# ekimb/rust-mdbg

Hardware: AMD Instinct MI355X
Metric: Gbases/s ingested to k-min-mer graph (higher is better)
Workload: dtype u64

## Files before the change

rust_mdbg_amd/csrc/owner.hip:

```cpp
#include "mdbg_dev.h"
__global__ void owner_thresholds_kernel(double bound, u32 k, u32 world, u64* __restrict__ thr) {
    const u32 r = threadIdx.x + 1;
    if (threadIdx.x == 0) thr[0] = 0;
    thr += OWNER_THR_AT;
    if (r >= world) return;
    const double x = -expm1(log1p(-(double)r / (double)world) / (double)k);
    double v = x * bound;
    thr[r - 1] = v >= 18446744073709549568.0 ? ~0ull : (u64)v;
}
void launch_owner_thresholds(double bound, u32 k, u32 world, u64* thr, hipStream_t s) {
    if (world > 1) hipLaunchKernelGGL(owner_thresholds_kernel, dim3(1), dim3(64), 0, s, bound, k, world, thr);
}

__global__ __launch_bounds__(256) void count_owned_windows_kernel(const u64* __restrict__ mh, const u32* __restrict__ mread, const u64* __restrict__ roff, u64 i0, u64 i1,
                                                                  u32 k, u32 world, const u64* thr, u32 rank, u64* __restrict__ out) {
    constexpr int WPT = 4;
    const u64 b0 = i0 + (u64)blockIdx.x * (256 * WPT);
    u32 slot[WPT]; bool ok[WPT];
#pragma unroll
    for (int u = 0; u < WPT; ++u) { const u64 i = b0 + u * 256 + threadIdx.x; ok[u] = i < i1; slot[u] = ok[u] ? mread[i] : 0; }
    u32 mine = 0;
#pragma unroll
    for (int u = 0; u < WPT; ++u) {
        const u64 i = b0 + u * 256 + threadIdx.x;
// ... 79 lines not shown
    if (threadIdx.x < world) hist[threadIdx.x] = 0;
    const u64 b0 = i0 + (u64)blockIdx.x * OWNL_SPAN;
    const OwnerSpec os{world, thr};
    const bool staged = k <= OWNL_LDS_MAX_K && thr != nullptr && world > 1;
    OwnerCodes oc{}; const u16* cur = nullptr; u32 p = 1;
    if (staged) {
        oc = owner_codes_of(os);
        u16* const ca = (u16*)sh_min;
        cur = span_min_codes([&](u32 t) { return mh[b0 + t]; }, [&](u32 t) { return b0 + t < i1; }, OWNL_SPAN + k - 1, k, oc, ca, ca + (OWNL_SPAN + k), p);
    } else __syncthreads();
#pragma unroll
    for (int u = 0; u < OWNL_SPAN / 256; ++u) {
        const u32 li = u * 256 + threadIdx.x;
        const u64 i = b0 + li;
        u32 o = 0xFFu;
        if (window_starts_at(mread, roff, i, i1, k)) {
            if (staged) { const u16 x = cur[li], y = cur[li + k - p]; o = owner_of_code(x < y ? x : y, oc); }
            else o = window_owner(mh + i, k, os);
            atomicAdd(&hist[o], 1u);
        }
        if (i < i1) owner_of[i - i0] = (u8)o;
    }
    __syncthreads();
    if (threadIdx.x < world) blk_cnt[(size_t)blockIdx.x * world + threadIdx.x] = hist[threadIdx.x];
}
void launch_owner_list_count(const u64* mh, const u32* mread, const u64* roff, u64 i0, u64 i1, u32 k, u32 world, const u64* thr, u32* blk_cnt, u8* owner_of, hipStream_t s) {
    if (i1 > i0) hipLaunchKernelGGL(owner_list_count_kernel, dim3((unsigned)((i1 - i0 + OWNL_SPAN - 1) / OWNL_SPAN)), dim3(256), owner_span_codes_lds(k), s, mh, mread, roff, i0, i1, k, world, thr, blk_cnt, owner_of);
}
__global__ __launch_bounds__(256) void owner_list_write_kernel(const u64* __restrict__ mh, const u32* __restrict__ mread, const u64* __restrict__ roff, u64 i0, u64 i1,
                                                               u32 k, u32 world, const u64* thr, u32 slot0, const u64* __restrict__ blk_off, OwnerBases bases, u32* __restrict__ list,
                                                               const u8* __restrict__ owner_of, u32 direct_owner, u32* __restrict__ direct_dst) {
    constexpr int NG = OWNL_SPAN / 64;
    __shared__ u32 grp[NG][OWNL_MAX_WORLD];
    for (int t = threadIdx.x; t < NG * (int)OWNL_MAX_WORLD; t += 256) ((u32*)grp)[t] = 0;
    __syncthreads();
    const u64 b0 = i0 + (u64)blockIdx.x * OWNL_SPAN;
    const int lane = threadIdx.x & 63, wv = threadIdx.x >> 6;
    constexpr u32 NONE = 0xFFFFFFFFu;
    u32 own[OWNL_SPAN / 256], rank[OWNL_SPAN / 256], slot_of[OWNL_SPAN / 256];
#pragma unroll
    for (int u = 0; u < OWNL_SPAN / 256; ++u) {
        const u64 i = b0 + u * 256 + threadIdx.x;
        u32 o = NONE, slot = 0;
        if (i < i1) { const u32 ob = owner_of[i - i0]; if (ob != 0xFFu) { o = ob; slot = mread[i]; } }
        u32 r = 0;
        for (u64 todo = __ballot(o != NONE); todo;) {
            const u32 oo = (u32)__shfl((int)o, __ffsll((unsigned long long)todo) - 1, 64);
            const u64 m = __ballot(o == oo);
            if (o == oo) { r = (u32)__popcll(m & ((1ull << lane) - 1)); if (r == 0) grp[u * 4 + wv][oo] = (u32)__popcll(m); }
            todo &= ~m;
        }
        own[u] = o; rank[u] = r; slot_of[u] = slot;
    }
    __syncthreads();
    if (threadIdx.x < world) { u32 run = 0; for (int g = 0; g < NG; ++g) { const u32 c = grp[g][threadIdx.x]; grp[g][threadIdx.x] = run; run += c; } }
    __syncthreads();
#pragma unroll
    for (int u = 0; u < OWNL_SPAN / 256; ++u) {
        const u32 o = own[u];
        if (o == NONE || (o == direct_owner && !direct_dst)) continue;
        const u64 i = b0 + u * 256 + threadIdx.x;
        const u64 at = blk_off[(size_t)blockIdx.x * world + o] + grp[u * 4 + wv][o] + rank[u];
        uint2* const e = o == direct_owner ? (uint2*)direct_dst + at : (uint2*)list + (bases.b[o] + at);
        *e = make_uint2((u32)(i - i0), slot_of[u] - slot0);
    }
}
void launch_owner_list_write(const u64* mh, const u32* mread, const u64* roff, u64 i0, u64 i1, u32 k, u32 world, const u64* thr, u32 slot0, const u64* blk_off, const OwnerBases& bases, u32* list, const u8* owner_of, hipStream_t s,
                             u32 direct_owner = 0xFFFFFFFFu, u32* direct_dst = nullptr) {
    if (i1 > i0) hipLaunchKernelGGL(owner_list_write_kernel, dim3((unsigned)((i1 - i0 + OWNL_SPAN - 1) / OWNL_SPAN)), dim3(256), 0, s, mh, mread, roff, i0, i1, k, world, thr, slot0, blk_off, bases, list, owner_of, direct_owner, direct_dst);
}

struct SegBuckets { u64 start[OWNL_MAX_WORLD + 1]; u64 base[OWNL_MAX_WORLD]; u64 lim[OWNL_MAX_WORLD]; u32 n; u32 skip; };
__device__ inline u32 seg_bucket_of(const SegBuckets& B, u64 j) {
    u32 lo = 0, hi = B.n - 1;
    while (lo < hi) { const u32 mid = (lo + hi + 1) >> 1; if (B.start[mid] <= j) lo = mid; else hi = mid - 1; }
    return lo;
}
__device__ inline u32 seg_add_of(const uint2* __restrict__ list, u64 j, u32 k, const SegBuckets& B, u32& b) {
    b = seg_bucket_of(B, j);
    if (b == B.skip) return 0;
    if (j && B.start[b] != j) { const u32 d = list[j].x - list[j - 1].x; if (d < k) return d; }
    return k;
}
constexpr u32 SEG_BLOCK = 4096;
__global__ __launch_bounds__(256) void seg_sums_kernel(const uint2* __restrict__ list, u64 n, u32 k, SegBuckets B, u64* __restrict__ block_sum) {
    __shared__ u32 ws[4];
    u32 v = 0;
#pragma unroll
    for (int q = 0; q < SEG_BLOCK / 256; ++q) { const u64 j = (u64)blockIdx.x * SEG_BLOCK + q * 256 + threadIdx.x; u32 b; if (j < n) v += seg_add_of(list, j, k, B, b); }
    for (int d = 32; d; d >>= 1) v += __shfl_down(v, d, 64);
    if ((threadIdx.x & 63) == 0) ws[threadIdx.x >> 6] = v;
    __syncthreads();
    if (threadIdx.x == 0) block_sum[blockIdx.x] = (u64)ws[0] + ws[1] + ws[2] + ws[3];
}
__global__ __launch_bounds__(256) void seg_pick_kernel(const uint2* __restrict__ list, u64 n, u32 k, SegBuckets B, const u64* __restrict__ block_base, const u64* __restrict__ total,
                                                       u64* __restrict__ out) {
    __shared__ u32 ws[4];
    const u32 bq = blockIdx.x;
    const u64 j1 = bq < B.n ? B.start[bq] : n;
    if (j1 >= n) { if (threadIdx.x == 0) out[bq] = total[0]; return; }
    const u64 j0 = j1 - j1 % SEG_BLOCK;
    u32 v = 0;
#pragma unroll
    for (int q = 0; q < SEG_BLOCK / 256; ++q) { const u64 j = j0 + q * 256 + threadIdx.x; u32 b; if (j < j1) v += seg_add_of(list, j, k, B, b); }
    for (int d = 32; d; d >>= 1) v += __shfl_down(v, d, 64);
    if ((threadIdx.x & 63) == 0) ws[threadIdx.x >> 6] = v;
    __syncthreads();
    if (threadIdx.x == 0) out[bq] = block_base[j0 / SEG_BLOCK] + ws[0] + ws[1] + ws[2] + ws[3];
}
void launch_seg_prefix(const u32* list, u64 n, u32 k, const SegBuckets& B, u64* scan_tmp, u64* carry, u64* picks, hipStream_t s) {
    if (!n) return;
    const u32 nb = (u32)((n + SEG_BLOCK - 1) / SEG_BLOCK);
    hipLaunchKernelGGL(seg_sums_kernel, dim3(nb), dim3(256), 0, s, (const uint2*)list, n, k, B, scan_tmp);
    hipLaunchKernelGGL(tile_scan_top_kernel, dim3(1), dim3(256), 0, s, nb, scan_tmp, carry);
    hipLaunchKernelGGL(seg_pick_kernel, dim3(B.n + 1), dim3(256), 0, s, (const uint2*)list, n, k, B, scan_tmp, carry, picks);
}
__global__ __launch_bounds__(256) void seg_copy_kernel(const uint2* __restrict__ list, u64 n, u32 k, SegBuckets B, const u64* __restrict__ block_base,
                                                       u64* __restrict__ store, u64* __restrict__ payload, u64 payload_n, u32 to_store) {
    __shared__ u32 lpre[256];
    __shared__ u64 laddr[256];
    __shared__ u32 tmp[8];
    u64 P0 = block_base[blockIdx.x];
#pragma unroll 1
    for (int q = 0; q < SEG_BLOCK / 256; ++q) {
        const u64 j = (u64)blockIdx.x * SEG_BLOCK + q * 256 + threadIdx.x;
        u32 a = 0, b = 0, x = 0;
        if (j < n) { a = seg_add_of(list, j, k, B, b); x = list[j].x; }
        u32 T;
        const u32 excl = block_excl_scan_256(a, tmp, T);
        u64 at = ~0ull;
        if (j < n && !((u64)x + k > B.lim[b] || P0 + excl + a > payload_n)) at = B.base[b] + x + (k - a);
        lpre[threadIdx.x] = j < n ? excl : 0xFFFFFFFFu;
        laddr[threadIdx.x] = at;
        __syncthreads();
        for (u32 e = threadIdx.x; e < T; e += 256) {
            u32 lo = 0, hi = 255;
#pragma unroll
            for (int st = 0; st < 8; ++st) { const u32 mid = (lo + hi + 1) >> 1; if (lpre[mid] <= e) lo = mid; else hi = mid - 1; }
            const u64 src = laddr[lo];
            if (src == ~0ull) continue;
            u64* const h = store + src + (e - lpre[lo]);
            u64* const pp = payload + P0 + e;
            if (to_store) *h = *pp; else *pp = *h;
        }
        P0 += T;
    }
}
void launch_seg_copy(const u32* list, u64 n, u32 k, const SegBuckets& B, const u64* scan_tmp, u64* store, u64* payload, u64 payload_n, bool to_store, hipStream_t s) {
    if (n) hipLaunchKernelGGL(seg_copy_kernel, dim3((unsigned)((n + SEG_BLOCK - 1) / SEG_BLOCK)), dim3(256), 0, s, (const uint2*)list, n, k, B, scan_tmp, store, payload, payload_n, to_store ? 1u : 0u);
}

__device__ inline bool listed_check(u64 j) { return (((u32)j * 0x9E3779B1u) >> 28) == 0; }
struct ListedBatch { u64 start, m0, m1, first_ordinal; const u32* list; u32 slot0, n_reads; };
__global__ __launch_bounds__(256) void insert_listed_entries_kernel(TableArgs T, const u64* __restrict__ mh, u32* __restrict__ mread, const u64* __restrict__ roff,
                                                                    u64 m0, u64 m1, const u32* __restrict__ list, u64 n, u32 slot0, u32 n_reads, u64 first_ordinal,
                                                                    u32* __restrict__ cap_err, const ListedBatch* __restrict__ multi, u32 n_multi) {
    if (cap_err[1]) return;
    const u64 j = (u64)blockIdx.x * blockDim.x + threadIdx.x;
    const u32 k = T.ks.k;
    bool ok = j < n;
    u64 i = 0, rs = 0; u32 slot = 0;
    u64 jl = j;
    if (multi) {
        const u64 jw0 = (u64)blockIdx.x * blockDim.x + (threadIdx.x & ~63u);
        u64 jw = ((u64)__builtin_amdgcn_readfirstlane((u32)(jw0 >> 32)) << 32) | (u64)__builtin_amdgcn_readfirstlane((u32)jw0);
        if (jw >= n) jw = n - 1;
        u32 lo = 0, hi = n_multi - 1;
        while (lo < hi) { const u32 mid = (lo + hi + 1) >> 1; if (multi[mid].start <= jw) lo = mid; else hi = mid - 1; }
        if (ok && multi[lo + 1].start <= j) {
            hi = n_multi - 1;
            while (lo < hi) { const u32 mid = (lo + hi + 1) >> 1; if (multi[mid].start <= j) lo = mid; else hi = mid - 1; }
        }
        const ListedBatch b = multi[lo];
        m0 = b.m0; m1 = b.m1; list = b.list; slot0 = b.slot0; n_reads = b.n_reads; first_ordinal = b.first_ordinal; jl = j - b.start;
    }
    if (ok) {
        const uint2 e = ((const uint2*)list)[jl];
        i = m0 + e.x; slot = slot0 + e.y; ok = e.y < n_reads && i + k <= m1;
    }
    const u64* const w = mh + i;
    bool rev = false; u64 h = 0;
    if (ok) {
        const u64 w_first = w[0], w_last = w[k - 1];
        rs = roff[slot]; const u64 re = roff[slot + 1];
        ok = i >= rs && re - rs > k && i + k <= re;
        if (ok) {
            rev = w_first != w_last ? w_first > w_last : window_reversed(w, k);
            u64 smallest;
            h = key_hash_window_hbm(w, k, rev, smallest);
            ok = owner_of_min(smallest, k, OwnerSpec{T.own_world, T.own_thr}) == T.own_rank;
        }
    }
    wave_count_add(ok, T.own_inserted);
    const u64 win = i - rs;
    if (ok && win > WIN_MASK) { *cap_err = 1; ok = false; }
    const u64 ord = ((first_ordinal + (slot - slot0)) << WIN_BITS) | win;
    bool claimed, found;
    const u64 s = upsert_wave_h(T, ok, (u32)i, i, w, k, rev, h, claimed, found);
    if (claimed) { mread[i] = slot; if (T.claim) T.claim[i] = 1; }
    if (found) {
        atomicAdd(&T.tab[s].count, 1u);
        push_ordinal(T, s, ord);
    }
}
static void launch_listed_entries(const TableArgs& T, const u64* mh, u32* mread, const u64* roff, u64 m0, u64 m1, const u32* list, u64 n, u32 slot0, u32 n_reads, u64 first_ordinal,
                                  u32* cap_err, const ListedBatch* multi, u32 n_multi, hipStream_t s) {
    hipLaunchKernelGGL(insert_listed_entries_kernel, dim3((unsigned)((n + 255) / 256)), dim3(256), 0, s, T, mh, mread, roff, m0, m1, list, n, slot0, n_reads, first_ordinal, cap_err, multi, n_multi);
}
__global__ __launch_bounds__(256) void list_segments_kernel(const u32* __restrict__ list, u64 n, u32 n_spans, u32* __restrict__ seg) {
    const u64 j = (u64)blockIdx.x * blockDim.x + threadIdx.x;
    if (j >= n) return;
    const u32 last = n_spans - 1;
    u32 b = list[2 * j] / OWNL_SPAN; if (b > last) b = last;
    int pb = -1;
    if (j) { u32 q = list[2 * j - 2] / OWNL_SPAN; if (q > last) q = last; pb = (int)q; }
    for (int q = pb + 1; q <= (int)b; ++q) seg[q] = (u32)j;
}
u32 owner_list_spans(u64 n_minimizers) { return (u32)((n_minimizers + OWNL_SPAN - 1) / OWNL_SPAN); }
void launch_list_segments(const u32* list, u64 n, u32 n_spans, u32* seg, hipStream_t s) {
    (void)hipMemsetD32Async((hipDeviceptr_t)seg, (int)(u32)n, (size_t)n_spans + 1, s);
    if (n && n_spans) hipLaunchKernelGGL(list_segments_kernel, dim3((unsigned)((n + 255) / 256)), dim3(256), 0, s, list, n, n_spans, seg);
}
static size_t listed_span_lds(const TableArgs& T) { return ((size_t)OWNL_SPAN + T.ks.k) * sizeof(u64) + OWNL_SPAN; }
__global__ __launch_bounds__(256) void insert_listed_span_kernel(TableArgs T, const u64* __restrict__ mh, u32* __restrict__ mread, const u64* __restrict__ roff,
                                                                 u64 m0, u64 m1, const u32* __restrict__ list, const u32* __restrict__ seg, u64 n, u32 slot0,
                                                                 u32 n_reads, u64 first_ordinal, u32* __restrict__ cap_err) {
    extern __shared__ u64 sh_keys[];
    if (cap_err[1]) return;
    const u32 q = blockIdx.x, k = T.ks.k;
    const u32 s0 = seg[q], s1 = seg[q + 1];
    const u64 b0 = m0 + (u64)q * OWNL_SPAN;
    u8* const cl = (u8*)(sh_keys + OWNL_SPAN + k);
    const u64 span_n = m1 - b0 < (u64)OWNL_SPAN ? m1 - b0 : (u64)OWNL_SPAN;
    if (s0 >= s1 || s1 > n) {
        if (T.claim) for (u32 li = threadIdx.x; li < span_n; li += 256) T.claim[b0 + li] = 0;
        return;
    }
    const u64 lim = b0 + OWNL_SPAN + k - 1 < m1 ? b0 + OWNL_SPAN + k - 1 : m1;
    for (u64 t = b0 + threadIdx.x; t < lim; t += 256) sh_keys[t - b0] = mh[t];
    if (T.claim) for (int u = threadIdx.x; u < OWNL_SPAN / 8; u += 256) ((u64*)cl)[u] = 0;
    __syncthreads();
    for (u32 base = s0; base < s1; base += 256) {
        const u32 j = base + threadIdx.x;
        bool ok = j < s1;
        u32 li = 0; u64 i = 0;
        u32 slot = 0; u64 rs = 0;
        if (ok) {
            const uint2 e = ((const uint2*)list)[j];
            li = e.x; ok = li / OWNL_SPAN == q && e.y < n_reads; li -= q * OWNL_SPAN; i = b0 + li; slot = slot0 + e.y;
        }
        if (ok) {
            rs = roff[slot]; const u64 re = roff[slot + 1];
            ok = i >= rs && re - rs > k && i + k <= re && (!listed_check(j) || window_owner(sh_keys + li, k, OwnerSpec{T.own_world, T.own_thr}) == T.own_rank);
        }
        wave_count_add(ok, T.own_inserted);
        const u64 win = i - rs;
        if (ok && win > WIN_MASK) { *cap_err = 1; ok = false; }
        const u64 ord = ((first_ordinal + (slot - slot0)) << WIN_BITS) | win;
        bool claimed, found;
        const u64 s = upsert_wave(T, ok, li, i, sh_keys + li, k, claimed, found);
        if (claimed) { mread[i] = slot; if (T.claim) cl[li] = 1; }
        if (found) {
            atomicAdd(&T.tab[s].count, 1u);
            push_ordinal(T, s, ord);
        }
    }
    if (T.claim) {
        __syncthreads();
        for (u32 li = threadIdx.x; li < span_n; li += 256) T.claim[b0 + li] = cl[li];
    }
}
constexpr u64 LISTED_SPAN_MIN = 150;
bool listed_per_entry(const TableArgs& T, u64 m0, u64 m1, u64 n, bool have_seg) {
    return !have_seg || listed_span_lds(T) > 64 * 1024 || n < (u64)owner_list_spans(m1 - m0) * LISTED_SPAN_MIN;
}
void launch_insert_listed(const TableArgs& T, const u64* mh, u32* mread, const u64* roff, u64 m0, u64 m1, const u32* list, const u32* seg, u64 n, u32 slot0,
                          u32 n_reads, u64 first_ordinal, u32* cap_err, hipStream_t s) {
    if (!n) return;
    if (!listed_per_entry(T, m0, m1, n, seg != nullptr))
        hipLaunchKernelGGL(insert_listed_span_kernel, dim3(owner_list_spans(m1 - m0)), dim3(256), listed_span_lds(T), s, T, mh, mread, roff, m0, m1, list, seg, n, slot0, n_reads, first_ordinal, cap_err);
    else
        launch_listed_entries(T, mh, mread, roff, m0, m1, list, n, slot0, n_reads, first_ordinal, cap_err, nullptr, 0u, s);
}
void launch_insert_listed_multi(const TableArgs& T, const u64* mh, u32* mread, const u64* roff, const ListedBatch* d_batches, u32 n_batches, u64 total, u32* cap_err, hipStream_t s) {
    if (!total) return;
    launch_listed_entries(T, mh, mread, roff, 0ull, 0ull, nullptr, total, 0u, 0u, 0ull, cap_err, d_batches, n_batches, s);
}
```

rust_mdbg_amd/csrc/table.hip:

```cpp
#include "mdbg_dev.h"

struct __attribute__((aligned(32))) Slot {
    u64 word;
    u64 m1;
    u64 m2;
    u32 count;
    u32 pad;
};
constexpr u64 EMPTY = ~0ull;
constexpr u64 HMUL = 0x9E3779B97F4A7C15ull;

struct KeySrc {
    const u64* mh;
    const u64* arena;
    u32 k;
};

__device__ inline u64 load_relaxed(const u64* p) { return __hip_atomic_load(p, __ATOMIC_RELAXED, __HIP_MEMORY_SCOPE_AGENT); }

__device__ inline u64 rep_elem(const KeySrc& ks, u64 word, u32 j) {
    const u32 rep = (u32)word;
    if (word & (1ull << 33)) return ks.arena[(u64)rep * (ks.k + 2) + j];
    return (word & (1ull << 32)) ? ks.mh[(u64)rep + ks.k - 1 - j] : ks.mh[(u64)rep + j];
}

__device__ inline bool window_reversed(const u64* __restrict__ w, u32 k) {
    for (u32 j = 0; j < k / 2 + 1 && j < k; ++j) {
        const u64 a = w[j], b = w[k - 1 - j];
        if (a < b) return false;
        if (a > b) return true;
    }
    return true;
}
template <class ElemFn>
__device__ inline u64 key_hash_fn(ElemFn elem, u32 k) {
    u64 h0 = 0x243F6A8885A308D3ull, h1 = 0x13198A2E03707344ull, h2 = 0xA4093822299F31D0ull, h3 = 0x082EFA98EC4E6C89ull;
    u32 j = 0;
    for (; j + 4 <= k; j += 4) {
        h0 = (h0 ^ elem(j)) * HMUL;     h0 ^= h0 >> 29;
        h1 = (h1 ^ elem(j + 1)) * HMUL; h1 ^= h1 >> 29;
        h2 = (h2 ^ elem(j + 2)) * HMUL; h2 ^= h2 >> 29;
        h3 = (h3 ^ elem(j + 3)) * HMUL; h3 ^= h3 >> 29;
    }
    if (j < k) { h0 = (h0 ^ elem(j)) * HMUL; h0 ^= h0 >> 29; }
    if (j + 1 < k) { h1 = (h1 ^ elem(j + 1)) * HMUL; h1 ^= h1 >> 29; }
    if (j + 2 < k) { h2 = (h2 ^ elem(j + 2)) * HMUL; h2 ^= h2 >> 29; }
    return fmix64(h0 ^ rol64(h1, 17) ^ rol64(h2, 31) ^ rol64(h3, 47));
}
__device__ inline u64 key_hash_window(const u64* __restrict__ w, u32 k, bool rev) {
    return key_hash_fn([&](u32 j) { return rev ? w[k - 1 - j] : w[j]; }, k);
}
__device__ inline u64 key_hash_window_hbm(const u64* __restrict__ w, u32 k, bool rev, u64& smallest) {
    u64 h[4] = {0x243F6A8885A308D3ull, 0x13198A2E03707344ull, 0xA4093822299F31D0ull, 0x082EFA98EC4E6C89ull};
    const u64* const p = rev ? w + (k - 1) : w;
    const long st = rev ? -1 : 1;
    u64 mn = ~0ull;
    for (u32 j0 = 0; j0 < k; j0 += 16) {
        u64 v[16];
#pragma unroll
        for (int t = 0; t < 16; ++t) { const u32 j = j0 + t < k ? j0 + t : k - 1; v[t] = p[st * (long)j]; }
#pragma unroll
        for (int t = 0; t < 16; ++t)
            if (j0 + t < k) { h[t & 3] = (h[t & 3] ^ v[t]) * HMUL; h[t & 3] ^= h[t & 3] >> 29; mn = v[t] < mn ? v[t] : mn; }
    }
    smallest = mn;
    return fmix64(h[0] ^ rol64(h[1], 17) ^ rol64(h[2], 31) ^ rol64(h[3], 47));
}
__device__ inline u64 key_hash_canon(const u64* __restrict__ key, u32 k) {
    return key_hash_fn([&](u32 j) { return key[j]; }, k);
}

struct TableArgs {
    Slot* tab; u64 cap;
    u64* mx;
    u32 A;
    u64* n_distinct;
    KeySrc ks;
    u32 own_world, own_rank;
    const u64* own_thr;
    u32* probe_err;
    u64* own_inserted;
    u64 fp_mask;
    unsigned long long* link_ctr;
    u32 no_chain;
    u8* claim;
};

__device__ inline u64 home_slot(u64 h, u64 cap) { return __umul64hi(h << 24, cap); }

__device__ inline void push_ordinal(const TableArgs& T, u64 s, u64 x) {
    Slot* e = T.tab + s;
    const u32 A = T.A;
    const u64* last = A == 1 ? &e->m1 : A == 2 ? &e->m2 : &T.mx[s * (A - 2) + (A - 3)];
    if (x > load_relaxed(last)) return;
    u64 carry = x;
    for (u32 lvl = 0; lvl < A && carry != EMPTY; ++lvl) {
        u64* m = lvl == 0 ? &e->m1 : lvl == 1 ? &e->m2 : &T.mx[s * (A - 2) + (lvl - 2)];
        const u64 old = atomicMin((unsigned long long*)m, (unsigned long long)carry);
        if (old > carry) carry = old;
    }
}

template <class EqFn>
__device__ inline u64 upsert_slot_from(const TableArgs& T, u64 h, u64 myword_lo, EqFn same_key, bool& claimed, u64 s, u64 probes);
template <class EqFn>
__device__ inline u64 upsert_slot(const TableArgs& T, u64 h, u64 myword_lo, EqFn same_key, bool& claimed) {
    return upsert_slot_from(T, h, myword_lo, same_key, claimed, home_slot(h, T.cap), 0);
}
template <class EqFn>
__device__ inline u64 upsert_slot_from(const TableArgs& T, u64 h, u64 myword_lo, EqFn same_key, bool& claimed, u64 s, u64 probes) {
    claimed = false;
    const u64 fp = (h >> 34) & T.fp_mask;
    const u64 myword = (fp << 34) | myword_lo;
    for (; probes <= T.cap; ++probes) {
        u64 w = load_relaxed(&T.tab[s].word);
        if (w == EMPTY) {
            const u64 old = atomicCAS((unsigned long long*)&T.tab[s].word, (unsigned long long)EMPTY, (unsigned long long)myword);
            if (old == EMPTY) { wave_agg_inc(T.n_distinct); claimed = true; return s; }
            w = old;
        }
        if ((w >> 34) == fp && same_key(w)) return s;
        s = s + 1 == T.cap ? 0 : s + 1;
    }
    *T.probe_err = 1;
    return ~0ull;
}
typedef u64 u64x2_a8 __attribute__((ext_vector_type(2), aligned(8)));
__device__ inline bool same_key_window(const KeySrc& ks, u64 w, const u64* wl, bool rev_mine) {
    const u32 k = ks.k, rep = (u32)w;
    const u64* rp; bool cross;
    if (w & (1ull << 33)) { rp = ks.arena + (u64)rep * (k + 2); cross = rev_mine; }
    else { rp = ks.mh + rep; cross = rev_mine != ((w & (1ull << 32)) != 0); }
    if (k < 8) {
        u64 diff = 0;
        for (u32 j = 0; j < k; ++j) diff |= rp[j] ^ wl[cross ? k - 1 - j : j];
        return !diff;
    }
    if (k >= 16) {
        for (u32 j = 0;; j += 16) {
            if (j + 16 > k) j = k - 16;
            u64x2_a8 a[8];
#pragma unroll
            for (int t = 0; t < 8; ++t) a[t] = *(const u64x2_a8*)(rp + j + 2 * t);
            u64 diff = 0;
            if (!cross) {
                const u64* m = wl + j;
#pragma unroll
                for (int t = 0; t < 8; ++t) diff |= (a[t].x ^ m[2 * t]) | (a[t].y ^ m[2 * t + 1]);
            } else {
                const u64* m = wl + (k - 16 - j);
#pragma unroll
                for (int t = 0; t < 8; ++t) diff |= (a[t].x ^ m[15 - 2 * t]) | (a[t].y ^ m[14 - 2 * t]);
            }
            if (diff) return false;
            if (j + 16 >= k) return true;
        }
    }
    for (u32 j = 0;; j += 8) {
        if (j + 8 > k) j = k - 8;
        const u64x2_a8 a0 = *(const u64x2_a8*)(rp + j), a1 = *(const u64x2_a8*)(rp + j + 2),
                       a2 = *(const u64x2_a8*)(rp + j + 4), a3 = *(const u64x2_a8*)(rp + j + 6);
        u64 diff;
        if (!cross) {
            const u64* m = wl + j;
            diff = (a0.x ^ m[0]) | (a0.y ^ m[1]) | (a1.x ^ m[2]) | (a1.y ^ m[3]) | (a2.x ^ m[4]) | (a2.y ^ m[5]) | (a3.x ^ m[6]) | (a3.y ^ m[7]);
        } else {
            const u64* m = wl + (k - 8 - j);
            diff = (a0.x ^ m[7]) | (a0.y ^ m[6]) | (a1.x ^ m[5]) | (a1.y ^ m[4]) | (a2.x ^ m[3]) | (a2.y ^ m[2]) | (a3.x ^ m[1]) | (a3.y ^ m[0]);
        }
        if (diff) return false;
        if (j + 8 >= k) return true;
    }
}

constexpr u32 OWNER_BINS = 65536, OWNER_THR_AT = 1, OWNER_TAB_AT = 64, OWNER_PARAM_WORDS = OWNER_TAB_AT + OWNER_BINS / 8;
struct OwnerSpec { u32 world; const u64* thr; };
__device__ inline u32 owner_of_min(u64 m, u32 k, OwnerSpec os);
__device__ inline u32 window_owner(const u64* __restrict__ w, u32 k, OwnerSpec os) {
    if (os.world <= 1) return 0;
    u64 m = w[0];
    for (u32 j = 1; j < k; ++j) { const u64 x = w[j]; m = x < m ? x : m; }
    return owner_of_min(m, k, os);
}
__device__ inline u32 owner_of_min(u64 m, u32 k, OwnerSpec os) {
    (void)k;
    if (os.world <= 1) return 0;
    if (!os.thr) return (u32)__umul64hi(fmix64(m), (u64)os.world);
    const u64 mul = os.thr[0];
    if (mul) {
        const u64 bin = __umul64hi(m, mul);
        const u32 o = ((const u8*)(os.thr + OWNER_TAB_AT))[bin < OWNER_BINS ? bin : OWNER_BINS - 1];
        return o < os.world ? o : os.world - 1;
    }
    const u64* const thr = os.thr + OWNER_THR_AT;
    u32 lo = 0, hi = os.world - 1;
    while (lo < hi) { const u32 mid = (lo + hi) >> 1; if (thr[mid] <= m) lo = mid + 1; else hi = mid; }
    return lo;
}

struct OwnerCodes { u64 mul; const u64* thr; u32 world; };
__device__ inline OwnerCodes owner_codes_of(OwnerSpec os) { OwnerCodes c; c.thr = os.thr; c.world = os.world; c.mul = os.thr ? os.thr[0] : 0; return c; }
__device__ inline u16 owner_code(u64 v, const OwnerCodes& c) {
    if (c.mul) { const u64 bin = __umul64hi(v, c.mul); return (u16)(bin < OWNER_BINS ? bin : OWNER_BINS - 1); }
    const u64* const thr = c.thr + OWNER_THR_AT;
    u32 lo = 0, hi = c.world - 1;
    while (lo < hi) { const u32 mid = (lo + hi) >> 1; if (thr[mid] <= v) lo = mid + 1; else hi = mid; }
    return (u16)lo;
}
__device__ inline u32 owner_of_code(u16 code, const OwnerCodes& c) {
    if (!c.mul) return code;
    const u32 o = ((const u8*)(c.thr + OWNER_TAB_AT))[code];
    return o < c.world ? o : c.world - 1;
}
template <class ValueFn, class ValidFn>
__device__ inline const u16* span_min_codes(ValueFn value, ValidFn valid, u32 nv, u32 k, const OwnerCodes& c, u16* a, u16* b, u32& p) {
    for (u32 t = threadIdx.x; t < nv; t += 256) a[t] = valid(t) ? owner_code(value(t), c) : (u16)0xFFFFu;
    __syncthreads();
    for (p = 1; 2 * p <= k; p *= 2) {
        for (u32 t = threadIdx.x; t < nv; t += 256) { const u16 x = a[t], y = t + p < nv ? a[t + p] : (u16)0xFFFFu; b[t] = x < y ? x : y; }
        __syncthreads();
        u16* const sw = a; a = b; b = sw;
    }
    return a;
}

__device__ inline u64 upsert_wave_h(const TableArgs& T, bool act, u32 li, u64 i, const u64* w, u32 k, bool rev, u64 h, bool& claimed, bool& found);
__device__ inline u64 upsert_wave(const TableArgs& T, bool act, u32 li, u64 i, const u64* w, u32 k, bool& claimed, bool& found) {
    bool rev = false; u64 h = 0;
    if (act) { rev = window_reversed(w, k); h = key_hash_window(w, k, rev); }
    return upsert_wave_h(T, act, li, i, w, k, rev, h, claimed, found);
}
__device__ inline u64 upsert_wave_h(const TableArgs& T, bool act, u32 li, u64 i, const u64* w, u32 k, bool rev, u64 h, bool& claimed, bool& found) {
    const int lane = threadIdx.x & 63;
    const u64 fp = (h >> 34) & T.fp_mask;
    const u64 myword_lo = ((u64)rev << 32) | (u64)(u32)i;
    auto eq = [&](u64 word) { return same_key_window(T.ks, word, w, rev); };
    u64 s = act ? home_slot(h, T.cap) : 0, word = EMPTY, probes = 0;
    claimed = false;
    bool cand = false;
    if (act) {
        for (; probes <= T.cap; ++probes) {
            u64 wv = load_relaxed(&T.tab[s].word);
            if (wv == EMPTY) {
                const u64 old = atomicCAS((unsigned long long*)&T.tab[s].word, (unsigned long long)EMPTY, (unsigned long long)((fp << 34) | myword_lo));
                if (old == EMPTY) { wave_agg_inc(T.n_distinct); claimed = true; break; }
                wv = old;
            }
            if ((wv >> 34) == fp) { word = wv; cand = true; break; }
            s = s + 1 == T.cap ? 0 : s + 1;
        }
        if (!claimed && !cand) { *T.probe_err = 1; s = ~0ull; }
    }
    const bool cross = rev != ((word & (1ull << 32)) != 0);
    const u32 rep = (u32)word;
    const u32 p_li = (u32)__shfl_up((int)li, 1, 64), p_rep = (u32)__shfl_up((int)rep, 1, 64);
    const int p_info = __shfl_up((int)((cand && !(word & (1ull << 33)) ? 1 : 0) | (cross ? 2 : 0)), 1, 64);
    const bool link = cand && !T.no_chain && lane > 0 && !(word & (1ull << 33)) && (p_info & 1) && p_li + 1 == li && ((p_info >> 1) & 1) == (int)cross &&
                      rep == (cross ? p_rep - 1u : p_rep + 1u);
    bool pass = false;
    if (cand) pass = link ? T.ks.mh[(u64)rep + (cross ? 0u : k - 1u)] == w[k - 1] : eq(word);
    const u64 heads = __ballot(!link), fails = __ballot(cand && !pass);
    found = pass;
    if (link && pass) {
        const int hp = 63 - __clzll((unsigned long long)(heads & ((2ull << lane) - 1ull)));
        found = ((fails >> hp) & ((2ull << (lane - hp)) - 1ull)) == 0;
    }
    if (T.link_ctr) { const u64 lm = __ballot(link && found); if (lane == 0 && lm) atomicAdd(T.link_ctr, (unsigned long long)__popcll(lm)); }
    if (cand && !found) {
        const bool skip = !link;
        s = upsert_slot_from(T, h, myword_lo, eq, claimed, skip ? (s + 1 == T.cap ? 0 : s + 1) : s, probes + (skip ? 1 : 0));
        found = !claimed && s != ~0ull;
    }
    return s;
}

constexpr int OWN_SPAN = 2048;
static size_t insert_windows_lds(const TableArgs& T) {
    const size_t codes = T.own_world > 1 && T.own_thr ? 2 * ((size_t)OWN_SPAN + T.ks.k) * sizeof(u16) : 0;
    return (OWN_SPAN + T.ks.k) * sizeof(u64) + OWN_SPAN * sizeof(u16) + 16 + OWN_SPAN + codes;
}
__global__ __launch_bounds__(256) void insert_windows_kernel(TableArgs T, const u64* __restrict__ mh, const u32* __restrict__ mread,
                                                                   const u64* __restrict__ roff, u64 i0, u64 i1, u32 slot0, u64 first_ordinal,
                                                                   u32* __restrict__ cap_err, const u64* __restrict__ i1_dev, u64 n_lim) {
    extern __shared__ u64 sh_keys[];
    if (cap_err[1]) return;
    if (i1_dev) { i1 = *i1_dev; if (i0 + (u64)blockIdx.x * OWN_SPAN >= i1) return; }
    const u32 k = T.ks.k;
    u16* const list = (u16*)(sh_keys + OWN_SPAN + k);
    u32* const n_own = (u32*)(list + OWN_SPAN);
    u8* const cl = (u8*)(n_own + 4);
    const u64 b0 = i0 + (u64)blockIdx.x * OWN_SPAN;
    const u64 lim = b0 + OWN_SPAN + k - 1 < i1 ? b0 + OWN_SPAN + k - 1 : i1;
    for (u64 t = b0 + threadIdx.x; t < lim; t += 256) sh_keys[t - b0] = mh[t];
    if (threadIdx.x == 0) *n_own = 0;
    if (T.claim) for (int u = threadIdx.x; u < OWN_SPAN / 8; u += 256) ((u64*)cl)[u] = 0;
    __syncthreads();
    const bool by_codes = T.own_world > 1 && T.own_thr != nullptr;
    const u16* mc = nullptr; u32 pc = 1; OwnerCodes oc{};
    if (by_codes) {
        u16* const ca = (u16*)(cl + OWN_SPAN);
        oc = owner_codes_of(OwnerSpec{T.own_world, T.own_thr});
        const u32 n_st = (u32)(lim - b0);
        mc = span_min_codes([&](u32 t) { return sh_keys[t]; }, [&](u32 t) { return t < n_st; }, OWN_SPAN + k - 1, k, oc, ca, ca + (OWN_SPAN + k), pc);
    }
#pragma unroll
    for (int u = 0; u < OWN_SPAN / 256; ++u) {
        const u32 li = u * 256 + threadIdx.x;
        const u64 i = b0 + li;
        bool mine = false;
        bool own = i + k <= i1;
        if (own && T.own_world > 1) {
            if (by_codes) { const u16 x = mc[li], y = mc[li + k - pc]; own = owner_of_code(x < y ? x : y, oc) == T.own_rank; }
            else own = window_owner(sh_keys + li, k, OwnerSpec{T.own_world, T.own_thr}) == T.own_rank;
        }
        if (own) {
            const u32 slot = mread[i];
            const u64 rs = roff[slot], re = roff[slot + 1];
            mine = re - rs > k && i + k <= re;
        }
        const u64 m = __ballot(mine);
        u32 base = 0;
        if ((threadIdx.x & 63) == 0 && m) base = atomicAdd(n_own, (u32)__popcll(m));
        base = __shfl(base, 0, 64);
        if (mine) list[base + __popcll(m & ((1ull << (threadIdx.x & 63)) - 1))] = (u16)li;
    }
    __syncthreads();
    const u32 n = *n_own;
    if (threadIdx.x == 0 && n && T.own_world > 1) atomicAdd((unsigned long long*)ctr_shard(T.own_inserted), (unsigned long long)n);
    for (u32 j0 = 0; j0 < n; j0 += 256) {
        const u32 j = j0 + threadIdx.x;
        bool act = j < n;
        const u32 li = act ? list[j] : 0u;
        const u64 i = b0 + li;
        u64 ord = 0;
        if (act) {
            const u32 slot = mread[i];
            const u64 win = i - roff[slot];
            if (win > WIN_MASK) { *cap_err = 1; act = false; }
            ord = ((first_ordinal + (slot - slot0)) << WIN_BITS) | win;
        }
        bool claimed, found;
        const u64 s = upsert_wave(T, act, li, i, sh_keys + li, k, claimed, found);
        if (claimed && T.claim) cl[li] = 1;
        if (found) {
            atomicAdd(&T.tab[s].count, 1u);
            push_ordinal(T, s, ord);
        }
    }
    if (T.claim) {
        __syncthreads();
        const u64 hi = i1 - b0 < (u64)OWN_SPAN ? i1 - b0 : (u64)OWN_SPAN;
        for (u32 li = threadIdx.x; li < hi && li < n_lim - (u64)blockIdx.x * OWN_SPAN; li += 256) T.claim[b0 + li] = cl[li];
    }
}
void launch_insert_windows(const TableArgs& T, const u64* mh, const u32* mread, const u64* roff, u64 i0, u64 i1, u32 slot0,
                           u64 first_ordinal, u64* n_windows, u32* cap_err, hipStream_t s, const u64* i1_dev = nullptr, u64 n_starts = 0) {
    if (i1 <= i0) return;
    (void)n_windows;
    const u64 n = n_starts ? n_starts : i1 - i0;
    hipLaunchKernelGGL(insert_windows_kernel, dim3((unsigned)((n + OWN_SPAN - 1) / OWN_SPAN)), dim3(256), insert_windows_lds(T), s, T, mh, mread, roff, i0, i1, slot0, first_ordinal, cap_err, i1_dev, n);
}

__global__ __launch_bounds__(256) void insert_records_kernel(TableArgs T, u64 r0, u64 r1, u64* __restrict__ n_windows) {
    const u64 r = r0 + (u64)blockIdx.x * blockDim.x + threadIdx.x;
    if (r >= r1) return;
    const u32 k = T.ks.k;
    const u64* key = T.ks.arena + r * (k + 2);
    const u64 h = key[k + 1];
    bool claimed;
    const u64 s = upsert_slot(T, h, (1ull << 33) | (u64)(u32)r, [&](u64 word) { return same_key_window(T.ks, word, key, false); }, claimed);
    if (claimed || s == ~0ull) return;
    atomicAdd(&T.tab[s].count, 1u);
    push_ordinal(T, s, key[k]);
    (void)n_windows;
}
void launch_insert_records(const TableArgs& T, u64 r0, u64 r1, u64* n_windows, hipStream_t s) {
    if (r1 <= r0) return;
    hipLaunchKernelGGL(insert_records_kernel, dim3((unsigned)((r1 - r0 + 255) / 256)), dim3(256), 0, s, T, r0, r1, n_windows);
}

__global__ void clear_table_kernel(Slot* __restrict__ tab, u64 cap, u64* __restrict__ mx, u64 n_mx, ZeroList z) {
    const u64 stride = (u64)gridDim.x * blockDim.x;
    {
        const u64 i0 = (u64)blockIdx.x * blockDim.x + threadIdx.x;
#pragma unroll
        for (int r = 0; r < 6; ++r) for (u64 i = i0; i < z.n[r]; i += stride) z.p[r][i] = 0;
        if (i0 == 0 && z.set_p) *z.set_p = z.set_v;
    }
    for (u64 i = (u64)blockIdx.x * blockDim.x + threadIdx.x; i < cap; i += stride) {
        uint4* p = (uint4*)(tab + i);
        p[0] = make_uint4(0xFFFFFFFFu, 0xFFFFFFFFu, 0xFFFFFFFFu, 0xFFFFFFFFu);
        p[1] = make_uint4(0xFFFFFFFFu, 0xFFFFFFFFu, 0u, 0u);
    }
    for (u64 i = (u64)blockIdx.x * blockDim.x + threadIdx.x; i < n_mx; i += stride) mx[i] = EMPTY;
}
void launch_clear_table(Slot* tab, u64 cap, u64* mx, u64 n_mx, hipStream_t s, const ZeroList* z = nullptr) {
    ZeroList none{};
    hipLaunchKernelGGL(clear_table_kernel, dim3(2048), dim3(256), 0, s, tab, cap, mx, n_mx, z ? *z : none);
}

__global__ void rehash_kernel(const Slot* __restrict__ old, u64 old_cap, const u64* __restrict__ old_mx, TableArgs T) {
    const u64 i = (u64)blockIdx.x * blockDim.x + threadIdx.x;
    if (i >= old_cap) return;
    const Slot e = old[i];
    if (e.word == EMPTY) return;
    const u64 h = key_hash_fn([&](u32 j) { return rep_elem(T.ks, e.word, j); }, T.ks.k);
    u64 s = home_slot(h, T.cap);
    for (;;) {
        const u64 oldw = atomicCAS((unsigned long long*)&T.tab[s].word, (unsigned long long)EMPTY, (unsigned long long)e.word);
        if (oldw == EMPTY) break;
        s = s + 1 == T.cap ? 0 : s + 1;
    }
    T.tab[s].m1 = e.m1; T.tab[s].m2 = e.m2; T.tab[s].count = e.count;
    for (u32 j = 0; j + 2 < T.A; ++j) T.mx[s * (T.A - 2) + j] = old_mx[i * (T.A - 2) + j];
}
void launch_rehash(const Slot* old, u64 old_cap, const u64* old_mx, const TableArgs& T, hipStream_t s) {
    hipLaunchKernelGGL(rehash_kernel, dim3((unsigned)((old_cap + 255) / 256)), dim3(256), 0, s, old, old_cap, old_mx, T);
}

__global__ __launch_bounds__(256) void reserve_check_kernel(const u64* __restrict__ distinct_shards, u64* __restrict__ n_distinct, const u64* __restrict__ batch_windows, u64 cap,
                                                            u32* __restrict__ too_small, const u64* __restrict__ carry, u64 store_cap, const u32* __restrict__ over_max) {
    __shared__ u64 ws[4];
    u64 v = 0;
    for (int i = threadIdx.x; i < CTR_SHARDS; i += 256) v += distinct_shards[i];
    for (int d = 32; d; d >>= 1) v += __shfl_down(v, d, 64);
    if ((threadIdx.x & 63) == 0) ws[threadIdx.x >> 6] = v;
    __syncthreads();
    if (threadIdx.x == 0) {
        const u64 nd = ws[0] + ws[1] + ws[2] + ws[3];
        *n_distinct = nd;
        const u64 n = nd + *batch_windows;
        bool skip = n + n / 2 + 1024 > cap;
        if (carry) skip = skip || *carry > store_cap || *carry >= 0xFFFFFFF0ull || (over_max && *over_max);
        *too_small = skip ? 1u : 0u;
    }
}
void launch_reserve_check(const u64* distinct_shards, u64* n_distinct, const u64* batch_windows, u64 cap, u32* too_small, hipStream_t s,
                          const u64* carry = nullptr, u64 store_cap = 0, const u32* over_max = nullptr) {
    hipLaunchKernelGGL(reserve_check_kernel, dim3(1), dim3(256), 0, s, distinct_shards, n_distinct, batch_windows, cap, too_small, carry, store_cap, over_max);
}

__global__ __launch_bounds__(1024) void count_reserve_kernel(const u64* __restrict__ roff, u32 slot0, u32 n_reads, u32 k, u64* __restrict__ batch_windows, u32* __restrict__ done,
                                                             const u64* __restrict__ distinct_shards, u64* __restrict__ n_distinct, u64 cap, u32* __restrict__ too_small,
                                                             const u64* __restrict__ carry, u64 store_cap, const u32* __restrict__ over_max) {
    __shared__ u64 ws[16];
    __shared__ u32 last;
    u64 w = 0;
    for (u32 r = blockIdx.x * blockDim.x + threadIdx.x; r < n_reads; r += gridDim.x * blockDim.x) { const u64 n = roff[slot0 + r + 1] - roff[slot0 + r]; if (n > k) w += n - k + 1; }
    for (int d = 32; d; d >>= 1) w += __shfl_down(w, d, 64);
    if ((threadIdx.x & 63) == 0) ws[threadIdx.x >> 6] = w;
    __syncthreads();
    if (threadIdx.x == 0) {
        u64 t = 0;
        for (int i = 0; i < 16; ++i) t += ws[i];
        if (t) atomicAdd((unsigned long long*)batch_windows, (unsigned long long)t);
        __threadfence();
        last = atomicAdd(done, 1u) + 1u == gridDim.x ? 1u : 0u;
    }
    __syncthreads();
    if (!last) return;
    __threadfence();
    u64 v = 0;
    for (int i = threadIdx.x; i < CTR_SHARDS; i += 1024) v += distinct_shards[i];
    for (int d = 32; d; d >>= 1) v += __shfl_down(v, d, 64);
    __syncthreads();
    if ((threadIdx.x & 63) == 0) ws[threadIdx.x >> 6] = v;
    __syncthreads();
    if (threadIdx.x == 0) {
        u64 nd = 0;
        for (int i = 0; i < 16; ++i) nd += ws[i];
        *n_distinct = nd;
        const u64 bw = __hip_atomic_load(batch_windows, __ATOMIC_RELAXED, __HIP_MEMORY_SCOPE_AGENT);
        const u64 n = nd + bw;
        bool skip = n + n / 2 + 1024 > cap;
        if (carry) skip = skip || *carry > store_cap || *carry >= 0xFFFFFFF0ull || (over_max && *over_max);
        *too_small = skip ? 1u : 0u;
        *done = 0;
    }
}
void launch_count_reserve(const u64* roff, u32 slot0, u32 n_reads, u32 k, u64* batch_windows, u32* done, const u64* distinct_shards, u64* n_distinct, u64 cap, u32* too_small,
                          const u64* carry, u64 store_cap, const u32* over_max, hipStream_t s) {
    hipLaunchKernelGGL(count_reserve_kernel, dim3(n_reads ? std::min<u32>(64u, (n_reads + 1023) / 1024) : 1), dim3(1024), 0, s, roff, slot0, n_reads, k, batch_windows, done, distinct_shards, n_distinct, cap,
                       too_small, carry, store_cap, over_max);
}

__global__ __launch_bounds__(256) void slice_check_kernel(const u64* __restrict__ distinct_shards, u64* __restrict__ n_distinct, u64 bound, u64 cap, u32* __restrict__ too_small,
                                                          u64* __restrict__ fail_at, u64 id) {
    __shared__ u64 ws[4];
    if (*too_small) return;
    u64 v = 0;
    for (int i = threadIdx.x; i < CTR_SHARDS; i += 256) v += distinct_shards[i];
    for (int d = 32; d; d >>= 1) v += __shfl_down(v, d, 64);
    if ((threadIdx.x & 63) == 0) ws[threadIdx.x >> 6] = v;
    __syncthreads();
    if (threadIdx.x == 0) {
        const u64 nd = ws[0] + ws[1] + ws[2] + ws[3];
        *n_distinct = nd;
        const u64 n = nd + bound;
        if (n + n / 2 + 1024 > cap) { *fail_at = id; *too_small = 1u; }
    }
}
void launch_slice_check(const u64* distinct_shards, u64* n_distinct, u64 bound, u64 cap, u32* too_small, u64* fail_at, u64 id, hipStream_t s) {
    hipLaunchKernelGGL(slice_check_kernel, dim3(1), dim3(256), 0, s, distinct_shards, n_distinct, bound, cap, too_small, fail_at, id);
}

__global__ __launch_bounds__(1024) void count_windows_kernel(const u64* __restrict__ roff, u32 slot0, u32 n_reads, u32 k, u64* __restrict__ out) {
    __shared__ u64 ws[16];
    const u32 r = blockIdx.x * blockDim.x + threadIdx.x;
    u64 w = 0;
    if (r < n_reads) { const u64 n = roff[slot0 + r + 1] - roff[slot0 + r]; if (n > k) w = n - k + 1; }
    for (int d = 32; d; d >>= 1) w += __shfl_down(w, d, 64);
    if ((threadIdx.x & 63) == 0) ws[threadIdx.x >> 6] = w;
    __syncthreads();
    if (threadIdx.x == 0) {
        u64 t = 0;
        for (int i = 0; i < 16; ++i) t += ws[i];
        if (t) atomicAdd((unsigned long long*)out, (unsigned long long)t);
    }
}
void launch_count_windows(const u64* roff, u32 slot0, u32 n_reads, u32 k, u64* out, hipStream_t s) {
    if (!n_reads) return;
    hipLaunchKernelGGL(count_windows_kernel, dim3((n_reads + 1023) / 1024), dim3(1024), 0, s, roff, slot0, n_reads, k, out);
}

template <class EqFn>
__device__ inline u64 find_slot(const TableArgs& T, u64 h, EqFn same_key) {
// ... 46 lines not shown
```

Baseline: 2548.

## Fetch slot word and m2 in one 16-byte probe load to skip reload

Moves m2 next to the key word in the hash slot and reads both with one 16-byte inline-asm global load while probing. When a repeated key is found with A==2, the early-exit test in ordinal pushing uses the copy from the probe instead of a second relaxed load. The insert kernels also get an amdgpu_waves_per_eu(5) occupancy hint. The inline asm issues its own s_waitcnt vmcnt(0), which can block the compiler from overlapping other loads. The copied m2 can also be stale by the time it is compared.

```diff
diff --git a/rust_mdbg_amd/csrc/owner.hip b/rust_mdbg_amd/csrc/owner.hip
--- a/rust_mdbg_amd/csrc/owner.hip
+++ b/rust_mdbg_amd/csrc/owner.hip
@@ -255,7 +255,7 @@
 
 __device__ inline bool listed_check(u64 j) { return (((u32)j * 0x9E3779B1u) >> 28) == 0; }
 struct ListedBatch { u64 start, m0, m1, first_ordinal; const u32* list; u32 slot0, n_reads; };
-__global__ __launch_bounds__(256) void insert_listed_entries_kernel(TableArgs T, const u64* __restrict__ mh, u32* __restrict__ mread, const u64* __restrict__ roff,
+__global__ __launch_bounds__(256) __attribute__((amdgpu_waves_per_eu(5))) void insert_listed_entries_kernel(TableArgs T, const u64* __restrict__ mh, u32* __restrict__ mread, const u64* __restrict__ roff,
                                                                     u64 m0, u64 m1, const u32* __restrict__ list, u64 n, u32 slot0, u32 n_reads, u64 first_ordinal,
                                                                     u32* __restrict__ cap_err, const ListedBatch* __restrict__ multi, u32 n_multi) {
     if (cap_err[1]) return;
@@ -298,13 +298,10 @@
     const u64 win = i - rs;
     if (ok && win > WIN_MASK) { *cap_err = 1; ok = false; }
     const u64 ord = ((first_ordinal + (slot - slot0)) << WIN_BITS) | win;
-    bool claimed, found;
-    const u64 s = upsert_wave_h(T, ok, (u32)i, i, w, k, rev, h, claimed, found);
+    bool claimed, found; u64 m2_copy;
+    const u64 s = upsert_wave_h(T, ok, (u32)i, i, w, k, rev, h, claimed, found, m2_copy);
     if (claimed) { mread[i] = slot; if (T.claim) T.claim[i] = 1; }
-    if (found) {
-        atomicAdd(&T.tab[s].count, 1u);
-        push_ordinal(T, s, ord);
-    }
+    if (found) repeated_sighting(T, s, ord, m2_copy);
 }
 static void launch_listed_entries(const TableArgs& T, const u64* mh, u32* mread, const u64* roff, u64 m0, u64 m1, const u32* list, u64 n, u32 slot0, u32 n_reads, u64 first_ordinal,
                                   u32* cap_err, const ListedBatch* multi, u32 n_multi, hipStream_t s) {
@@ -360,13 +357,10 @@
         const u64 win = i - rs;
         if (ok && win > WIN_MASK) { *cap_err = 1; ok = false; }
         const u64 ord = ((first_ordinal + (slot - slot0)) << WIN_BITS) | win;
-        bool claimed, found;
-        const u64 s = upsert_wave(T, ok, li, i, sh_keys + li, k, claimed, found);
+        bool claimed, found; u64 m2_copy;
+        const u64 s = upsert_wave(T, ok, li, i, sh_keys + li, k, claimed, found, m2_copy);
         if (claimed) { mread[i] = slot; if (T.claim) cl[li] = 1; }
-        if (found) {
-            atomicAdd(&T.tab[s].count, 1u);
-            push_ordinal(T, s, ord);
-        }
+        if (found) repeated_sighting(T, s, ord, m2_copy);
     }
     if (T.claim) {
         __syncthreads();
diff --git a/rust_mdbg_amd/csrc/table.hip b/rust_mdbg_amd/csrc/table.hip
--- a/rust_mdbg_amd/csrc/table.hip
+++ b/rust_mdbg_amd/csrc/table.hip
@@ -2,11 +2,12 @@
 
 struct __attribute__((aligned(32))) Slot {
     u64 word;
+    u64 m2;
     u64 m1;
-    u64 m2;
     u32 count;
     u32 pad;
 };
+static_assert(sizeof(Slot) == 32 && offsetof(Slot, word) == 0 && offsetof(Slot, m2) == 8, "probe_slot reads {word, m2} as the slot's first 16 bytes");
 constexpr u64 EMPTY = ~0ull;
 constexpr u64 HMUL = 0x9E3779B97F4A7C15ull;
 
@@ -17,6 +18,16 @@
 };
 
 __device__ inline u64 load_relaxed(const u64* p) { return __hip_atomic_load(p, __ATOMIC_RELAXED, __HIP_MEMORY_SCOPE_AGENT); }
+struct Probe { u64 word, m2; };
+typedef u32 u32x4 __attribute__((ext_vector_type(4)));
+__device__ inline Probe probe_slot(const Slot* e) {
+    u32x4 v;
+    asm volatile("global_load_dwordx4 %0, %1, off sc1\n\ts_waitcnt vmcnt(0)" : "=v"(v) : "v"(e) : "memory");
+    Probe p;
+    p.word = ((u64)v.y << 32) | v.x; p.m2 = ((u64)v.w << 32) | v.z;
+    return p;
+}
+constexpr u64 M2_UNKNOWN = ~0ull;
 
 __device__ inline u64 rep_elem(const KeySrc& ks, u64 word, u32 j) {
     const u32 rep = (u32)word;
@@ -88,11 +99,12 @@
 
 __device__ inline u64 home_slot(u64 h, u64 cap) { return __umul64hi(h << 24, cap); }
 
-__device__ inline void push_ordinal(const TableArgs& T, u64 s, u64 x) {
+__device__ inline void repeated_sighting(const TableArgs& T, u64 s, u64 x, u64 m2_copy) {
     Slot* e = T.tab + s;
     const u32 A = T.A;
-    const u64* last = A == 1 ? &e->m1 : A == 2 ? &e->m2 : &T.mx[s * (A - 2) + (A - 3)];
-    if (x > load_relaxed(last)) return;
+    atomicAdd(&e->count, 1u);
+    const u64 last = A == 2 ? m2_copy : load_relaxed(A == 1 ? &e->m1 : &T.mx[s * (A - 2) + (A - 3)]);
+    if (x > last) return;
     u64 carry = x;
     for (u32 lvl = 0; lvl < A && carry != EMPTY; ++lvl) {
         u64* m = lvl == 0 ? &e->m1 : lvl == 1 ? &e->m2 : &T.mx[s * (A - 2) + (lvl - 2)];
@@ -102,24 +114,26 @@
 }
 
 template <class EqFn>
-__device__ inline u64 upsert_slot_from(const TableArgs& T, u64 h, u64 myword_lo, EqFn same_key, bool& claimed, u64 s, u64 probes);
+__device__ inline u64 upsert_slot_from(const TableArgs& T, u64 h, u64 myword_lo, EqFn same_key, bool& claimed, u64& m2_copy, u64 s, u64 probes);
 template <class EqFn>
-__device__ inline u64 upsert_slot(const TableArgs& T, u64 h, u64 myword_lo, EqFn same_key, bool& claimed) {
-    return upsert_slot_from(T, h, myword_lo, same_key, claimed, home_slot(h, T.cap), 0);
+__device__ inline u64 upsert_slot(const TableArgs& T, u64 h, u64 myword_lo, EqFn same_key, bool& claimed, u64& m2_copy) {
+    return upsert_slot_from(T, h, myword_lo, same_key, claimed, m2_copy, home_slot(h, T.cap), 0);
 }
 template <class EqFn>
-__device__ inline u64 upsert_slot_from(const TableArgs& T, u64 h, u64 myword_lo, EqFn same_key, bool& claimed, u64 s, u64 probes) {
+__device__ inline u64 upsert_slot_from(const TableArgs& T, u64 h, u64 myword_lo, EqFn same_key, bool& claimed, u64& m2_copy, u64 s, u64 probes) {
     claimed = false;
+    m2_copy = M2_UNKNOWN;
     const u64 fp = (h >> 34) & T.fp_mask;
     const u64 myword = (fp << 34) | myword_lo;
     for (; probes <= T.cap; ++probes) {
-        u64 w = load_relaxed(&T.tab[s].word);
+        const Probe p = probe_slot(T.tab + s);
+        u64 w = p.word, m2 = p.m2;
         if (w == EMPTY) {
             const u64 old = atomicCAS((unsigned long long*)&T.tab[s].word, (unsigned long long)EMPTY, (unsigned long long)myword);
             if (old == EMPTY) { wave_agg_inc(T.n_distinct); claimed = true; return s; }
-            w = old;
-        }
-        if ((w >> 34) == fp && same_key(w)) return s;
+            w = old; m2 = M2_UNKNOWN;
+        }
+        if ((w >> 34) == fp && same_key(w)) { m2_copy = m2; return s; }
         s = s + 1 == T.cap ? 0 : s + 1;
     }
     *T.probe_err = 1;
@@ -224,29 +238,31 @@
     return a;
 }
 
-__device__ inline u64 upsert_wave_h(const TableArgs& T, bool act, u32 li, u64 i, const u64* w, u32 k, bool rev, u64 h, bool& claimed, bool& found);
-__device__ inline u64 upsert_wave(const TableArgs& T, bool act, u32 li, u64 i, const u64* w, u32 k, bool& claimed, bool& found) {
+__device__ inline u64 upsert_wave_h(const TableArgs& T, bool act, u32 li, u64 i, const u64* w, u32 k, bool rev, u64 h, bool& claimed, bool& found, u64& m2_copy);
+__device__ inline u64 upsert_wave(const TableArgs& T, bool act, u32 li, u64 i, const u64* w, u32 k, bool& claimed, bool& found, u64& m2_copy) {
     bool rev = false; u64 h = 0;
     if (act) { rev = window_reversed(w, k); h = key_hash_window(w, k, rev); }
-    return upsert_wave_h(T, act, li, i, w, k, rev, h, claimed, found);
-}
-__device__ inline u64 upsert_wave_h(const TableArgs& T, bool act, u32 li, u64 i, const u64* w, u32 k, bool rev, u64 h, bool& claimed, bool& found) {
+    return upsert_wave_h(T, act, li, i, w, k, rev, h, claimed, found, m2_copy);
+}
+__device__ inline u64 upsert_wave_h(const TableArgs& T, bool act, u32 li, u64 i, const u64* w, u32 k, bool rev, u64 h, bool& claimed, bool& found, u64& m2_copy) {
     const int lane = threadIdx.x & 63;
     const u64 fp = (h >> 34) & T.fp_mask;
     const u64 myword_lo = ((u64)rev << 32) | (u64)(u32)i;
     auto eq = [&](u64 word) { return same_key_window(T.ks, word, w, rev); };
     u64 s = act ? home_slot(h, T.cap) : 0, word = EMPTY, probes = 0;
     claimed = false;
+    m2_copy = M2_UNKNOWN;
     bool cand = false;
     if (act) {
         for (; probes <= T.cap; ++probes) {
-            u64 wv = load_relaxed(&T.tab[s].word);
+            const Probe p = probe_slot(T.tab + s);
+            u64 wv = p.word, m2 = p.m2;
             if (wv == EMPTY) {
                 const u64 old = atomicCAS((unsigned long long*)&T.tab[s].word, (unsigned long long)EMPTY, (unsigned long long)((fp << 34) | myword_lo));
                 if (old == EMPTY) { wave_agg_inc(T.n_distinct); claimed = true; break; }
-                wv = old;
+                wv = old; m2 = M2_UNKNOWN;
             }
-            if ((wv >> 34) == fp) { word = wv; cand = true; break; }
+            if ((wv >> 34) == fp) { word = wv; m2_copy = m2; cand = true; break; }
             s = s + 1 == T.cap ? 0 : s + 1;
         }
         if (!claimed && !cand) { *T.probe_err = 1; s = ~0ull; }
@@ -268,7 +284,7 @@
     if (T.link_ctr) { const u64 lm = __ballot(link && found); if (lane == 0 && lm) atomicAdd(T.link_ctr, (unsigned long long)__popcll(lm)); }
     if (cand && !found) {
         const bool skip = !link;
-        s = upsert_slot_from(T, h, myword_lo, eq, claimed, skip ? (s + 1 == T.cap ? 0 : s + 1) : s, probes + (skip ? 1 : 0));
+        s = upsert_slot_from(T, h, myword_lo, eq, claimed, m2_copy, skip ? (s + 1 == T.cap ? 0 : s + 1) : s, probes + (skip ? 1 : 0));
         found = !claimed && s != ~0ull;
     }
     return s;
@@ -279,7 +295,7 @@
     const size_t codes = T.own_world > 1 && T.own_thr ? 2 * ((size_t)OWN_SPAN + T.ks.k) * sizeof(u16) : 0;
     return (OWN_SPAN + T.ks.k) * sizeof(u64) + OWN_SPAN * sizeof(u16) + 16 + OWN_SPAN + codes;
 }
-__global__ __launch_bounds__(256) void insert_windows_kernel(TableArgs T, const u64* __restrict__ mh, const u32* __restrict__ mread,
+__global__ __launch_bounds__(256) __attribute__((amdgpu_waves_per_eu(5))) void insert_windows_kernel(TableArgs T, const u64* __restrict__ mh, const u32* __restrict__ mread,
                                                                    const u64* __restrict__ roff, u64 i0, u64 i1, u32 slot0, u64 first_ordinal,
                                                                    u32* __restrict__ cap_err, const u64* __restrict__ i1_dev, u64 n_lim) {
     extern __shared__ u64 sh_keys[];
@@ -339,13 +355,10 @@
             if (win > WIN_MASK) { *cap_err = 1; act = false; }
             ord = ((first_ordinal + (slot - slot0)) << WIN_BITS) | win;
         }
-        bool claimed, found;
-        const u64 s = upsert_wave(T, act, li, i, sh_keys + li, k, claimed, found);
+        bool claimed, found; u64 m2_copy;
+        const u64 s = upsert_wave(T, act, li, i, sh_keys + li, k, claimed, found, m2_copy);
         if (claimed && T.claim) cl[li] = 1;
-        if (found) {
-            atomicAdd(&T.tab[s].count, 1u);
-            push_ordinal(T, s, ord);
-        }
+        if (found) repeated_sighting(T, s, ord, m2_copy);
     }
     if (T.claim) {
         __syncthreads();
@@ -367,11 +380,10 @@
     const u32 k = T.ks.k;
     const u64* key = T.ks.arena + r * (k + 2);
     const u64 h = key[k + 1];
-    bool claimed;
-    const u64 s = upsert_slot(T, h, (1ull << 33) | (u64)(u32)r, [&](u64 word) { return same_key_window(T.ks, word, key, false); }, claimed);
+    bool claimed; u64 m2_copy;
+    const u64 s = upsert_slot(T, h, (1ull << 33) | (u64)(u32)r, [&](u64 word) { return same_key_window(T.ks, word, key, false); }, claimed, m2_copy);
     if (claimed || s == ~0ull) return;
-    atomicAdd(&T.tab[s].count, 1u);
-    push_ordinal(T, s, key[k]);
+    repeated_sighting(T, s, key[k], m2_copy);
     (void)n_windows;
 }
 void launch_insert_records(const TableArgs& T, u64 r0, u64 r1, u64* n_windows, hipStream_t s) {
```

After: 2576 (median of 6 runs). Within noise of the previous version (+1.1%).
